# dronefreak/CABiNet

Hardware: NVIDIA B200
Metric: images/sec at 1024x1024 (MNv3-L) (higher is better)
Workload: dtype bf16

## Files before the change

cabinet_b200/_lib.py:

```python

from __future__ import annotations

import ctypes as C
import subprocess
from pathlib import Path

PKG = Path(__file__).resolve().parent
LIB_PATH = PKG / "libcabinet_b200.so"
CSRC = PKG / "csrc"

F32, BF16, F16 = 0, 1, 2
ACT_NONE, ACT_RELU, ACT_HSWISH, ACT_HSIGMOID, ACT_SIGMOID = 0, 1, 2, 3, 4

_p, _i, _ll, _f = C.c_void_p, C.c_int, C.c_longlong, C.c_float

SIGNATURES = {
    "cabinet_last_error": ([], C.c_char_p),
    "cabinet_abi_version": ([], _i),
    "cabinet_device_info": ([C.POINTER(_i)] * 3, _i),
    "cabinet_debug_flags": ([_i], _i),
    "cabinet_debug_read": ([_p, _i], _i),
    "cabinet_conv2d_simt": ([_p, _i, _ll, _ll, _ll, _ll, _ll, _p, _i, _ll, _ll, _ll, _p, _p, _ll, _p, _i, _ll, _ll,
                             _i, _i, _i, _i, _i, _i, _i, _i, _i, _i, _i, _i, _i, _f, _p], _i),
    "cabinet_conv_tc": ([_p, _ll, _i, _i, _i, _i, _p, _i, _i, _i, _i, _i, _p, _p, _ll, _p, _i, _ll, _i, _i, _i, _p], _i),
    "cabinet_conv_tc_dt": ([_p, _ll, _i, _i, _i, _i, _p, _i, _i, _i, _i, _i, _p, _p, _ll, _p, _i, _ll, _i, _i, _i, _i, _p],
                           _i),
    "cabinet_conv_tc_view": ([_p, _ll, _i, _i, _i, _i, _p, _i, _i, _i, _i, _p, _p, _ll, _i, _i, _ll, _ll, _ll, _p], _i),
    "cabinet_conv_tc_view_dt": ([_p, _ll, _i, _i, _i, _i, _p, _i, _i, _i, _i, _p, _p, _ll, _i, _i, _ll, _ll, _ll, _i, _p], _i),
    "cabinet_conv_tc_se": ([_p, _ll, _i, _i, _i, _i, _p, _i, _p, _i, _i, _i, _i, _i, _p, _p, _ll, _p, _i, _ll, _i, _i, _i,
                            _p], _i),
    "cabinet_conv_tc_split_act": ([_p, _ll, _i, _i, _i, _i, _p, _i, _i, _i, _i, _i, _p, _p, _i, _ll, _i, _i, _i, _i, _p], _i),
    "cabinet_conv_tc_imgw": ([_p, _ll, _i, _i, _i, _i, _p, _ll, _i, _i, _i, _i, _i, _p, _p, _ll, _p, _i, _ll, _i, _i, _i,
                              _p], _i),
    "cabinet_conv_tc_imgw_dt": ([_p, _ll, _i, _i, _i, _i, _p, _ll, _i, _i, _i, _i, _i, _p, _p, _ll, _p, _i, _ll, _i, _i, _i,
                                 _i, _p], _i),
    "cabinet_conv_tc_up": ([_p, _ll, _i, _i, _i, _i, _p, _i, _i, _i, _i, _i, _p, _p, _i, _i, _p, _ll, _i, _i, _i, _p], _i),
    "cabinet_gate_scale_weights": ([_p, _i, _f, _p, _p, _p, _p, _i, _i, _i, _p, _p, _i, _i, _i, _i, _i, _p], _i),
    "cabinet_scale_weights": ([_p, _p, _p, _i, _i, _i, _i, _i, _i, _p], _i),
    "cabinet_stem_tc": ([_p, _i, _i, _i, _p, _p, _p, _ll, _p, _ll, _i, _i, _p], _i),
    "cabinet_stem_tc2": ([_p, _i, _i, _i, _p, _p, _ll, _p, _ll, _i, _i, _p], _i),
    "cabinet_dwconv": ([_p, _ll, _p, _p, _p, _ll, _i, _i, _i, _i, _i, _i, _i, _i, _i, _i, _p, _p], _i),
    "cabinet_dwconv_tma": ([_p, _ll, _p, _p, _p, _ll, _i, _i, _i, _i, _i, _i, _i, _i, _i, _p, _p], _i),
    "cabinet_dwconv_tma_dt": ([_p, _ll, _p, _p, _p, _ll, _i, _i, _i, _i, _i, _i, _i, _i, _i, _p, _i, _p], _i),
    "cabinet_mbconv_noexpand_fused": ([_p, _ll, _p, _p, _p, _p, _p, _ll, _i, _i, _i, _i, _i, _p], _i),
    "cabinet_mbconv_fused": ([_p, _ll, _i, _i, _i, _i, _p, _p, _i, _i, _i, _i, _i, _p, _p, _i, _i, _p, _ll, _i, _i, _p,
                              _p], _i),
    "cabinet_mbconv_t": ([_p, _ll, _i, _i, _i, _i, _p, _p, _i, _i, _i, _i, _i, _p, _p, _i, _i, _p, _ll, _i, _i, _p, _p,
                          _p], _i),
    "cabinet_expand_sums": ([_p, _ll, _i, _i, _i, _i, _p, _p, _i, _i, _i, _i, _p, _p], _i),
    "cabinet_gate_mlp": ([_p, _f, _p, _p, _p, _p, _p, _i, _i, _i, _i, _p], _i),
    "cabinet_gate_fc": ([_p, _f, _p, _p, _p, _i, _i, _i, _i, _i, _p], _i),
    "cabinet_scale_act": ([_p, _ll, _i, _p, _i, _ll, _i, _i, _i, _p], _i),
    "cabinet_psp_pool": ([_p, _ll, _i, _p, _i, _i, _i, _i, _p, _ll, _p], _i),
    "cabinet_psp_concat": ([_p, _ll, _p, _p, _ll, _i, _i, _i, _i, _i, _p], _i),
    "cabinet_softmax_rows": ([_p, _p, _i, _ll, _i, _p], _i),
    "cabinet_attention_tc": ([_p, _ll, _p, _ll, _p, _ll, _p, _p, _ll, _i, _i, _i, _f, _p], _i),
    "cabinet_cab_combine": ([_p, _p, _p, _p, _ll, _p, _i, _ll, _i, _p], _i),
    "cabinet_channel_sum": ([_p, _ll, _i, _i, _ll, _i, _p, _p, _ll, _p], _i),
    "cabinet_bilinear_nhwc": ([_p, _ll, _i, _p, _ll, _i, _i, _i, _i, _i, _i, _i, _p], _i),
    "cabinet_upsample_logits_nchw": ([_p, _i, _i, _i, _i, _p, _i, _i, _i, _p], _i),
    "cabinet_upsample_argmax": ([_p, _i, _i, _i, _i, _p, _i, _i, _p, _i, _i, _p, _p], _i),
    "cabinet_normalize_u8": ([_p, _p, _i, _i, _i, _f, _f, _f, _f, _f, _f, _p], _i),
    "cabinet_confusion_hist": ([_p, _i, _p, _i, _ll, _i, _i, _p, _p], _i),
    "cabinet_upsample_softmax_accum": ([_p, _p, _i, _i, _i, _i, _i, _i, _p, _ll, _ll, _ll, _i, _i, _i, _i, _p, _p, _f,
                                        _p], _i),
    "cabinet_prob_resize_accum": ([_p, _i, _i, _i, _i, _i, _i, _i, _i, _p, _i, _i, _p], _i),
    "cabinet_argmax_hist_nchw": ([_p, _i, _i, _ll, _p, _p, _i, _i, _p, _p], _i),
    "cabinet_ohem_workspace_bytes": ([], _ll),
    "cabinet_train_scratch_floats": ([_ll, _i, _i], _ll),
    "cabinet_pack_conv_weight": ([_p, _i, _i, _i, _i, _p, _i, _i, _i, _i, _p], _i),
    "cabinet_pack_conv_weight_parity": ([_p, _i, _i, _i, _i, _i, _i, _i, _i, _i, _p, _i, _i, _p], _i),
    "cabinet_pack_conv_weight_parity_dt": ([_p, _i, _i, _i, _i, _i, _i, _i, _i, _i, _p, _i, _i, _i, _p], _i),
    "cabinet_pack_dw_weight": ([_p, _i, _i, _i, _p, _p], _i),
    "cabinet_im2col_nchw": ([_p, _i, _i, _i, _i, _i, _i, _i, _p, _ll, _p], _i),
    "cabinet_im2col_nchw_dt": ([_p, _i, _i, _i, _i, _i, _i, _i, _p, _ll, _i, _p], _i),
    "cabinet_embed_filter": ([_p, _i, _i, _i, _i, _p, _ll, _i, _p], _i),
    "cabinet_bn_train_stats": ([_p, _ll, _i, _ll, _i, _p, _p, _f, _f, _p, _p, _p, _p, _p], _i),
    "cabinet_affine_act": ([_p, _ll, _i, _p, _p, _p, _f, _p, _ll, _p, _ll, _i, _ll, _ll, _i, _i, _p], _i),
    "cabinet_bn_train_backward": ([_p, _ll, _p, _ll, _i, _p, _i, _p, _p, _p, _ll, _ll, _i, _i, _p, _p], _i),
    "cabinet_bn_frozen_stats": ([_p, _p, _p, _p, _f, _i, _p, _p], _i),
    "cabinet_bn_frozen_backward": ([_p, _ll, _p, _ll, _i, _p, _i, _p, _p, _p, _ll, _ll, _i, _i, _p, _p], _i),
    "cabinet_stem_dgrad": ([_p, _ll, _p, _ll, _i, _p, _p, _p, _i, _i, _i, _i, _i, _p], _i),
    "cabinet_gate_scale_backward": ([_p, _ll, _p, _ll, _i, _p, _f, _i, _p, _i, _ll, _i, _p, _p], _i),
    "cabinet_gate_apply_backward": ([_p, _ll, _p, _ll, _i, _p, _f, _p, _f, _i, _p, _ll, _i, _ll, _i, _i, _p], _i),
    "cabinet_gate_mlp_backward": ([_p, _f, _p, _p, _p, _p, _p, _i, _i, _i, _i, _p, _p, _p, _p, _p, _p, _p], _i),
    "cabinet_col_sum": ([_p, _ll, _i, _ll, _i, _p, _i, _p, _p], _i),
    "cabinet_conv_dgrad": ([_p, _ll, _i, _p, _i, _ll, _ll, _p, _ll, _i, _i, _i, _i, _i, _i, _i, _i, _i, _i, _i, _i, _p], _i),
    "cabinet_conv_wgrad_scratch_floats": ([_i, _i, _i, _i, _i, _i, _i], _ll),
    "cabinet_conv_wgrad": ([_p, _ll, _i, _p, _i, _ll, _ll, _ll, _ll, _p, _i, _i, _i, _i, _i, _i, _i, _i, _i, _i, _i, _p,
                            _p], _i),
    "cabinet_conv_wgrad_tc_scratch_floats": ([_i, _i, _i, _i, _i, _i, _i, _i, _i], _ll),
    "cabinet_conv_wgrad_tc": ([_p, _ll, _p, _ll, _p, _i, _i, _i, _i, _i, _i, _i, _i, _i, _p, _p], _i),
    "cabinet_conv_wgrad_tc_dt": ([_p, _ll, _p, _ll, _p, _i, _i, _i, _i, _i, _i, _i, _i, _i, _p, _i, _p], _i),
# ... 57 lines not shown
```

cabinet_b200/engine.py:

```python

from __future__ import annotations

import math
from dataclasses import dataclass
from typing import Optional

import torch

from . import _lib
from ._lib import ACT_HSIGMOID, ACT_HSWISH, ACT_NONE, ACT_RELU, ACT_SIGMOID, BF16, F16, F32, check
from .constants import BN_EPS


_DTYPE_CODES = {torch.float32: F32, torch.bfloat16: BF16, torch.float16: F16}


def dtype_code(dtype: torch.dtype) -> int:
    code = _DTYPE_CODES.get(dtype)
    if code is None:
        raise TypeError(f"cabinet_b200 kernels take float32, bfloat16 or float16 tensors, got {dtype}")
    return code


@dataclass
# ... 121 lines not shown
    return o


def _out_size(n, k, s, p):
    return (n + 2 * p - k) // s + 1


class Engine:
    PACKED_ATTRS = ("stem", "blocks", "last", "stem_tc", "sb1", "sb2", "sb3", "sb4", "conva", "to_q", "to_k", "to_v",
                    "psp_k", "psp_v", "proj_out", "local", "gamma", "convb", "b1", "b4", "key_ch", "qkv", "ffm_blk",
                    "ffm_gate", "head_conv", "head_out", "ffm_sb", "low_fold", "stem_tc2")

    def __init__(self, model, precision: str = "bf16", packed: Optional[dict] = None):
        if precision not in ("bf16", "fp32"):
            raise ValueError(f"precision must be 'bf16' or 'fp32', got {precision!r}")
        p0 = next(model.parameters())
        if not p0.is_cuda:
            raise RuntimeError("cabinet_b200 engine needs the model on a CUDA device (no CPU path)")
        self.lib = _lib.load()
        self.dev = p0.device
        self.precision = precision
        self.tdt = torch.bfloat16 if precision == "bf16" else torch.float32
        self.dt = BF16 if precision == "bf16" else F32
        self.n_classes = model.n_classes
        self.stamp = None
        self.launches = 0
        self.use_tc = precision == "bf16"
        self.debug = False
        self.stages = {}
        self.trace, self.trace_filter = None, None
        self.fuse_mbconv = True
        self.se_from_sums = True
        self.use_stem2 = True
        self.t_small_s2 = False
        self.t_k5s2 = True
        self.use_mbconv_t = True
        self.fold_se_relu = True
        self.fold_ffm = True
        self.fold_low_up = False
        self.reverse_layers = frozenset()
        self.fuse_se = False
        self.fuse_se_blocks = frozenset({"mobile.f12", "mobile.f13"})
        self.use_cuda_graph = False
        self.sub_batch = 0
        self._graphs = {}
        self._pool = None
        self._graph_seen = {}
        self.dual_stream = False
        self._side = None
        self._scratch = []
        self.branch_overlap = True
        self._branch_streams, self._branch_events = [], {}
        self.sb_overlap = False
        if packed is not None:
            missing = [a for a in self.PACKED_ATTRS if a not in packed]
            if missing:
                raise ValueError(f"packed weights lack {missing}")
            for a in self.PACKED_ATTRS:
                setattr(self, a, _from_plain(packed[a]))
            self.gamma = model.ab.a2block.gamma.detach().float().contiguous()
        else:
            with torch.no_grad():
                self._pack(model)
                for a in self.PACKED_ATTRS:
                    setattr(self, a, _map_tensors(getattr(self, a), lambda t: t.to(self.dev)))

    def packed_state(self) -> dict:
        return {a: _to_plain(getattr(self, a)) for a in self.PACKED_ATTRS}

    def _pack(self, m):
        wd = self.tdt
        f32 = torch.float32
        mob = m.mobile
        self.stem = ConvLayer(mob.features[0][0], mob.features[0][1], ACT_HSWISH, f32, "mobile.stem")
        self.blocks = []
        for bi, blk in enumerate(list(mob.features)[1:], 1):
            s, c = blk.spec, blk.conv
            act = ACT_HSWISH if s["hs"] else ACT_RELU
            e = dict(spec=s, act=act)
            if s["expand"]:
                e["pw1"] = ConvLayer(c[0], c[1], act, wd, f"mobile.f{bi}.expand")
                e["dw"] = DwLayer(c[3], c[4], ACT_NONE if s["se"] else act, f"mobile.f{bi}.dw")
                se, pw2, bn2 = c[5], c[7], c[8]
                if self.precision == "bf16":
                    dwl, kk, nc = e["dw"], e["dw"].k ** 2, -(-e["dw"].c // 64)
                    aux = torch.zeros((nc * 64, kk + 2), dtype=f32, device=dwl.w.device)
                    aux[: dwl.c, :kk] = dwl.w.t()
                    aux[: dwl.c, kk + 1] = dwl.b
                    e["aux"] = aux.view(nc, 64, kk + 2).permute(0, 2, 1).contiguous()
                    p1 = e["pw1"]
                    if p1.cin % 8 == 0 and p1.cin % 64 <= 56 and p1.cin <= 248:
                        wb = torch.zeros((-(-p1.cout // 16) * 16, (p1.cin // 64 + 1) * 64), dtype=f32, device=dwl.w.device)
                        wb[: p1.cout, : p1.cin] = p1.tc[: p1.cout, 0, : p1.cin].float()
                        hi = p1.b.to(torch.bfloat16).float()
                        wb[: p1.cout, p1.cin], wb[: p1.cout, p1.cin + 1] = hi, p1.b - hi
                        e["w1b"] = wb.to(torch.bfloat16).contiguous()
                        ch = 64 if dwl.c <= 64 else 128
                        nct = 1 if dwl.c <= 64 else -(-dwl.c // 128)
                        flat = torch.zeros((nct * ch, wb.shape[1]), dtype=f32, device=dwl.w.device)
                        flat[: dwl.c] = wb[: dwl.c]
                        e["w1t"] = (flat.view(nct, ch, -1).repeat(1, 128 // ch, 1).reshape(nct * 128, -1)
                                    .to(torch.bfloat16).contiguous())
                        fa = torch.zeros((nct * ch, kk + 1), dtype=f32, device=dwl.w.device)
                        fa[: dwl.c, :kk] = dwl.w.t()
                        fa[: dwl.c, kk] = dwl.b
                        e["auxt"] = fa.view(nct, ch, kk + 1).repeat(1, 128 // ch, 1).permute(0, 2, 1).contiguous()
# ... 78 lines not shown
    def _run(self, kernel: str, layer: str, nbytes: int, flops: int, fn, *args):
        nbytes, fused_bytes = nbytes if isinstance(nbytes, tuple) else (nbytes, nbytes)
        tr = self.trace
        if tr is not None and (self.trace_filter is None or kernel in self.trace_filter):
            e0, e1 = torch.cuda.Event(enable_timing=True), torch.cuda.Event(enable_timing=True)
            e0.record()
            rc = fn(*args)
            e1.record()
            tr.append((kernel, layer, nbytes, flops, e0, e1, fused_bytes))
        else:
            rc = fn(*args)
        check(rc, f"{kernel}[{layer}]")
        self.launches += 1

    def new(self, N, H, W, C, dtype=None) -> Map:
        t = torch.empty((N, H, W, C), dtype=dtype or self.tdt, device=self.dev)
        return Map(t, N, H, W, C, C)

    def conv(self, x: Map, L: ConvLayer, out: Optional[Map] = None, res: Optional[Map] = None, out_dtype=None,
             nchw_input: Optional[torch.Tensor] = None, a_scale: Optional[torch.Tensor] = None, a_act: int = 0) -> Map:
        if nchw_input is not None:
            N, _, H, W = nchw_input.shape
            xptr, xdt, xes = nchw_input.data_ptr(), F32, 4
            sxn, sxh, sxw, sxc = 3 * H * W, W, 1, H * W
            cin = 3
        else:
            N, H, W, cin = x.N, x.H, x.W, x.C
            xptr, xdt, xes = x.ptr, x.dt, x.t.element_size()
            sxn, sxh, sxw, sxc = H * W * x.ld, W * x.ld, x.ld, 1
        assert cin == L.cin, (L.name, cin, L.cin)
        OH, OW = _out_size(H, L.kh, L.stride, L.pad), _out_size(W, L.kw, L.stride, L.pad)
        if out is None:
            out = self.new(N, OH, OW, L.cout, out_dtype)
        assert (out.N, out.H, out.W, out.C) == (N, OH, OW, L.cout), L.name
        M = N * OH * OW
        nbytes = (N * H * W * cin * xes + M * L.cout * out.t.element_size() + L.w.numel() * L.w.element_size()
                  + (M * L.cout * res.t.element_size() if res is not None else 0))
        flops = 2 * M * L.cout * L.cin * L.kh * L.kw
        if (self.use_tc and L.tc is not None and nchw_input is None and x.dt == BF16 and x.ld % 8 == 0
                and x.off % 8 == 0 and (L.stride == 1 or (H >= 2 and W >= 2))
                and (out.dt == F32 or (out.ld % 8 == 0 and out.off % 8 == 0))):
            self._conv_tc(x, L, out, res, OH, OW, nbytes, flops, a_scale, a_act)
            return out
        assert a_scale is None, "the SE prologue exists on the tcgen05 path only"
        wdt = BF16 if L.w.dtype == torch.bfloat16 else F32
        self._run("conv2d_simt", L.name, nbytes, flops, self.lib.cabinet_conv2d_simt,
                  xptr, xdt, sxn, sxh, sxw, sxc, 0, L.w.data_ptr(), wdt, L.w.shape[1], 1, 0, L.b.data_ptr(),
                  res.ptr if res is not None else None, res.ld if res is not None else 0,
                  out.ptr, out.dt, out.ld, 0, 1, N, H, W, cin, L.cout, L.kh, L.kw, L.stride, L.pad, OH, OW, L.act,
                  1.0, self.stream)
        return out

    REVERSE_TILES = 0x100

    def _conv_tc(self, x: Map, L: ConvLayer, out: Map, res: Optional[Map], OH, OW, nbytes, flops, a_scale=None, a_act=0):
        self._run("conv_tc", L.name, nbytes, flops, self.lib.cabinet_conv_tc_se, x.ptr, x.ld, x.N, x.H, x.W, x.C,
                  a_scale.data_ptr() if a_scale is not None else None, a_act,
                  L.tc.data_ptr(), L.cout, L.kh, L.kw, L.stride, L.pad, L.b.data_ptr(),
                  res.ptr if res is not None else None, res.ld if res is not None else 0, out.ptr, out.dt, out.ld,
                  OH, OW, L.act | (self.REVERSE_TILES if L.name in self.reverse_layers else 0), self.stream)

    def dwconv(self, x: Map, L: DwLayer, gap: Optional[torch.Tensor] = None):
        p = (L.k - 1) // 2
        OH, OW = _out_size(x.H, L.k, L.stride, p), _out_size(x.W, L.k, L.stride, p)
        out = self.new(x.N, OH, OW, x.C)
        es = x.t.element_size()
        nbytes = x.N * x.C * (x.H * x.W + OH * OW) * es + L.w.numel() * 4
        flops = 2 * x.N * OH * OW * x.C * L.k * L.k
        if self.use_tc and x.dt == BF16 and x.ld % 8 == 0 and x.off % 8 == 0:
            self._run("dwconv_tma", L.name, nbytes, flops, self.lib.cabinet_dwconv_tma, x.ptr, x.ld, L.w.data_ptr(),
                      L.b.data_ptr(), out.ptr, out.ld, x.N, x.H, x.W, x.C, L.k, L.stride, OH, OW,
                      L.act | (self.REVERSE_TILES if L.name in self.reverse_layers else 0),
                      gap.data_ptr() if gap is not None else None, self.stream)
            return out, True
        self._run("dwconv", L.name, nbytes, flops, self.lib.cabinet_dwconv, x.ptr, x.ld, L.w.data_ptr(),
                  L.b.data_ptr(), out.ptr, out.ld, x.dt, x.N, x.H, x.W, x.C, L.k, L.stride, OH, OW, L.act, None,
                  self.stream)
        if gap is not None:
            self.channel_sum(out, gap, L.name)
        return out, False

    def channel_sum(self, x: Map, out: torch.Tensor, name: str, scratch: Optional[torch.Tensor] = None):
        if scratch is None:
            scratch = torch.zeros(128 + x.N * 64 * x.C, dtype=torch.float32, device=self.dev)
            self.launches += 1
        self._run("channel_sum", name, 0, 0, self.lib.cabinet_channel_sum, x.ptr, x.ld, x.dt, x.N, x.H * x.W, x.C,
                  out.data_ptr(), scratch.data_ptr(), scratch.numel() * 4, self.stream)

    class _Branch:

        def __init__(self, eng, i):
            self.eng, self.i = eng, i

        def __enter__(self):
            eng = self.eng
            if not eng.branch_overlap or eng.trace is not None or torch.device(eng.dev).type != "cuda":
                self.ctx = None
                return lambda t: None
            self.main = torch.cuda.current_stream(eng.dev)
            while len(eng._branch_streams) <= self.i:
                eng._branch_streams.append(torch.cuda.Stream(eng.dev))
            side = eng._branch_streams[self.i]
            ev = torch.cuda.Event()
            ev.record(self.main)
            side.wait_event(ev)
            self.ctx = torch.cuda.stream(side)
            self.ctx.__enter__()
            return lambda t: t.record_stream(self.main)

        def __exit__(self, *a):
            if self.ctx is not None:
                eng = self.eng
                ev = torch.cuda.Event()
# ... 116 lines not shown
        cat = self.new(x.N, x.H, x.W, 5 * x.C)
        self._run("psp_concat", L.name, 0, 0, self.lib.cabinet_psp_concat, x.ptr, x.ld, pooled.data_ptr(), cat.ptr,
                  cat.ld, x.dt, x.N, x.H, x.W, x.C, self.stream)
        return self.conv(cat, L)

    def attention(self, q: Map, k: Map, v: Map) -> Map:
        N, Lq, d = q.N, q.H * q.W, q.C
        es = q.t.element_size()
        ctx = self.new(q.N, q.H, q.W, d)
        if self.use_tc and d == 128 and q.dt == BF16 and all(m.ld % 8 == 0 and m.off % 8 == 0 for m in (q, k, v)):
            vt = torch.empty((N, d, -(-Lq // 8) * 8), dtype=torch.bfloat16, device=self.dev)
            self._run("attention_tc", "cab.attention", 4 * N * Lq * d * es, 4 * N * Lq * Lq * d,
                      self.lib.cabinet_attention_tc, q.ptr, q.ld, k.ptr, k.ld, v.ptr, v.ld, vt.data_ptr(), ctx.ptr,
                      ctx.ld, N, Lq, d, float(d) ** -0.5, self.stream)
            self.launches += 1
            return ctx
        s = torch.empty((N, Lq, Lq), dtype=torch.float32, device=self.dev)
        self._run("conv2d_simt", "cab.qk", 2 * N * Lq * d * es, 2 * N * Lq * Lq * d, self.lib.cabinet_conv2d_simt,
                  q.ptr, q.dt, 0, 0, q.ld, 1, Lq * q.ld, k.ptr, k.dt, k.ld, 1, Lq * k.ld, None, None, 0,
                  s.data_ptr(), F32, Lq, Lq * Lq, N, 1, 1, Lq, d, Lq, 1, 1, 1, 0, 1, Lq, ACT_NONE, float(d) ** -0.5,
                  self.stream)
        p = torch.empty((N, Lq, Lq), dtype=self.tdt, device=self.dev)
        self._run("softmax_rows", "cab.softmax", 0, 0, self.lib.cabinet_softmax_rows, s.data_ptr(), p.data_ptr(),
                  self.dt, N * Lq, Lq, self.stream)
        self._run("conv2d_simt", "cab.pv", 2 * N * Lq * d * es, 2 * N * Lq * Lq * d, self.lib.cabinet_conv2d_simt,
                  p.data_ptr(), self.dt, 0, 0, Lq, 1, Lq * Lq, v.ptr, v.dt, 1, v.ld, Lq * v.ld, None, None, 0,
                  ctx.ptr, ctx.dt, ctx.ld, Lq * ctx.ld, N, 1, 1, Lq, Lq, d, 1, 1, 1, 0, 1, Lq, ACT_NONE, 1.0,
                  self.stream)
        return ctx

    def bilinear(self, x: Map, out: Map, name: str):
        nbytes = x.N * x.C * (x.H * x.W * x.t.element_size() + out.H * out.W * out.t.element_size())
        self._run("bilinear_nhwc", name, nbytes, 0, self.lib.cabinet_bilinear_nhwc, x.ptr, x.ld, x.dt, out.ptr, out.ld,
                  out.dt, x.N, x.H, x.W, x.C, out.H, out.W, self.stream)

    def _trunk(self, x: torch.Tensor, need_aux: bool = True):
        if x.dtype != torch.float32 or not x.is_contiguous():
            x = x.float().contiguous()
        if x.device != self.dev:
            raise RuntimeError(f"input on {x.device}, model on {self.dev}")
        N, _, H, W = x.shape
        self.launches = 0
        dev, C = self.dev, self.n_classes
        n_se = sum(1 for b in self.blocks if "se" in b)
        kc = self.key_ch
        n_gap, n_psp, n_ffm = (2 * n_se + 1) * N * 1024, 128 + N * (110 + 256 * kc), 128 + N * 64 * 256
        zeros_all = torch.zeros(n_gap + 2 * n_psp + n_ffm, dtype=torch.float32, device=dev)
        gap_all = zeros_all[:n_gap].view(2 * n_se + 1, N * 1024)
        self._scratch = [zeros_all[n_gap + i * n_psp: n_gap + (i + 1) * n_psp] for i in range(2)]
        ffm_scratch = zeros_all[n_gap + 2 * n_psp:]
        self.launches += 1

        fused_stems = self.use_tc and self.stem_tc is not None and W % 4 == 0
        if fused_stems:
            OH2, OW2 = (H - 1) // 2 + 1, (W - 1) // 2 + 1
            s1, f0 = self.new(N, OH2, OW2, 64), self.new(N, OH2, OW2, 16)
            nbytes = x.numel() * 4 + (s1.t.numel() + f0.t.numel()) * 2 + 80 * 192 * 2
            if self.use_stem2 and self.stem_tc2 is not None:
                self._run("stem_tc", "sb.conv1+mobile.stem", nbytes, 2 * N * OH2 * OW2 * (64 * 147 + 16 * 27),
                          self.lib.cabinet_stem_tc2, x.data_ptr(), N, H, W, self.stem_tc2.data_ptr(), s1.ptr, s1.ld,
                          f0.ptr, f0.ld, OH2, OW2, self.stream)
            else:
                self._run("stem_tc", "sb.conv1+mobile.stem", nbytes, 2 * N * OH2 * OW2 * (64 * 147 + 16 * 27),
                          self.lib.cabinet_stem_tc, x.data_ptr(), N, H, W, self.stem_tc[0].data_ptr(),
                          self.stem_tc[1].data_ptr(), s1.ptr, s1.ld, f0.ptr, f0.ld, OH2, OW2, self.stream)
        else:
            s1 = self.conv(None, self.sb1, nchw_input=x)
        H8, W8 = _out_size(_out_size(s1.H, 3, 2, 1), 3, 2, 1), _out_size(_out_size(s1.W, 3, 2, 1), 3, 2, 1)
        fold_low = (self.fold_low_up and self.use_tc and not self.debug and self.ffm_sb is not None
                    and self.ffm_sb.tc is not None and self.low_fold.tc is not None and self.sb4.cout == self.ffm_sb.cin)
        cat_ffm = self.new(N, H8, W8, self.sb4.cout if fold_low else 128 + 256)
        if self.sb_overlap:
            with self._branch(2) as joined:
                s2 = self.conv(s1, self.sb2)
                s3 = self.conv(s2, self.sb3)
                self.conv(s3, self.sb4, out=cat_ffm.slice(0, 128))
                joined(s1.t)
        else:
            s2 = self.conv(s1, self.sb2)
            s3 = self.conv(s2, self.sb3)
            self.conv(s3, self.sb4, out=cat_ffm.slice(0, 128))
        assert (s3.H, s3.W) == (H8, W8)

        f = f0 if fused_stems else self.conv(None, self.stem, nchw_input=x)
        gi = 0
        for e in self.blocks:
            s = e["spec"]
            if "fused_pw" in e and self.use_tc and f.ld % 8 == 0 and f.off % 8 == 0:
                o = self.new(f.N, f.H, f.W, s["out"])
                dw = e["dw"]
                es = f.t.element_size()
                self._run("mbconv_noexpand_fused", dw.name.replace(".dw", ""), 2 * f.N * f.H * f.W * f.C * es,
                          2 * f.N * f.H * f.W * f.C * (9 + f.C), self.lib.cabinet_mbconv_noexpand_fused, f.ptr, f.ld,
                          dw.w.data_ptr(), dw.b.data_ptr(), e["fused_pw"][0].data_ptr(), e["fused_pw"][1].data_ptr(),
                          o.ptr, o.ld, f.N, f.H, f.W, f.C, dw.act, self.stream)
                f = o
                continue
            fuse = (s["expand"] and self.fuse_mbconv and self.use_tc and f.dt == BF16 and f.ld % 8 == 0
                    and f.off % 8 == 0 and s["exp"] % 8 == 0 and ("se" in e or s["out"] <= 160) and "w1b" in e
                    and not e.get("nofuse")
                    and not (s["k"] == 5 and s["s"] == 2 and not (self.use_mbconv_t and self.t_k5s2 and "se" in e)))
            d = None
            gap_fixed = False
            if fuse and "se" in e and self.se_from_sums and self._se_from_sums_ok(f, e):
                try:
                    f = self.se_block_one_kernel(f, e, gap_all[2 * gi:2 * gi + 2].view(-1)[: 2 * N * s["exp"]])
                    gi += 1
                    continue
                except ValueError as err:
                    if "budget" not in str(err):
                        raise
                    e["no_sums"] = True
            if fuse:
                gap = None
                if "se" in e:
                    gap, gap_fixed = gap_all[2 * gi:2 * gi + 2].view(-1)[: 2 * N * s["exp"]], True
                pw2l = e["pw2"]
                fold_se = ("se" in e and self.fold_se_relu and e["act"] == ACT_RELU and not self.debug
                           and pw2l.tc is not None and pw2l.kh == 1 and (f.H // s["s"]) * (f.W // s["s"]) % 128 == 0
                           and f.H % s["s"] == 0 and f.W % s["s"] == 0)
                try:
                    d = self.mbconv_fused(f, e, gap, ACT_RELU if fold_se else None)
                except ValueError as err:
                    if "budget" not in str(err):
                        raise
                    e["nofuse"], fuse = True, False
            if fuse and "se" not in e:
                f = d
                continue
            h = self.conv(f, e["pw1"]) if s["expand"] and not fuse else f
            if "se" in e:
                if not fuse:
                    gap = gap_all[2 * gi:2 * gi + 2].view(-1)[: 2 * N * s["exp"]]
                    d, gap_fixed = self.dwconv(h, e["dw"], gap)
                gi += 1
# ... 293 lines not shown
```

include/cabinet_b200.h:

```cpp
#ifndef CABINET_B200_H
#define CABINET_B200_H

#include <stdint.h>

#ifdef __cplusplus
extern "C" {
#endif

#define CABINET_ABI_VERSION 2

enum { CABINET_OK = 0, CABINET_ERR_INVALID = 1, CABINET_ERR_CUDA = 2 };
enum { CABINET_F32 = 0, CABINET_BF16 = 1, CABINET_F16 = 2 };
enum {
    CABINET_ACT_NONE = 0,
    CABINET_ACT_RELU = 1,
    CABINET_ACT_HSWISH = 2,
    CABINET_ACT_HSIGMOID = 3,
    CABINET_ACT_SIGMOID = 4
};
#define CABINET_CONV_REVERSE_TILES 0x100

#define CABINET_GAP_FIXED_ONE 16777216.0f

typedef void* cabinet_stream_t;

const char* cabinet_last_error(void);
int cabinet_abi_version(void);
int cabinet_device_info(int* sm_count, int* cc_major, int* cc_minor);
int cabinet_debug_flags(int flags);
int cabinet_debug_read(long long* host_out, int n);

int cabinet_conv2d_simt(const void* x, int x_dtype, long long sxn, long long sxh, long long sxw, long long sxc,
                        long long x_batch_stride,
                        const void* w, int w_dtype, long long w_sco, long long w_sk, long long w_batch_stride,
                        const float* bias,
                        const void* res, long long ldres,
                        void* y, int y_dtype, long long ldy, long long y_batch_stride,
                        int batches, int N, int H, int W, int Cin, int Cout, int KH, int KW, int stride, int pad,
                        int OH, int OW, int act, float alpha, cabinet_stream_t stream);

int cabinet_conv_tc(const void* x, long long ldx, int N, int H, int W, int Cin, const void* w_packed, int Cout,
                    int KH, int KW, int stride, int pad, const float* bias, const void* res, long long ldres,
                    void* y, int y_dtype, long long ldy, int OH, int OW, int act, cabinet_stream_t stream);
int cabinet_conv_tc_dt(const void* x, long long ldx, int N, int H, int W, int Cin, const void* w_packed, int Cout,
                       int KH, int KW, int stride, int pad, const float* bias, const void* res, long long ldres,
                       void* y, int y_dtype, long long ldy, int OH, int OW, int act, int op_dtype, cabinet_stream_t stream);

int cabinet_conv_tc_view(const void* x, long long ldx, int N, int H, int W, int Cin, const void* w_packed, int Cout, int KH,
                         int KW, int pad, const float* bias, void* y, long long ldy, int OH, int OW, long long y_sw,
                         long long y_sh, long long y_sn, cabinet_stream_t stream);
int cabinet_conv_tc_view_dt(const void* x, long long ldx, int N, int H, int W, int Cin, const void* w_packed, int Cout, int KH,
                            int KW, int pad, const float* bias, void* y, long long ldy, int OH, int OW, long long y_sw,
                            long long y_sh, long long y_sn, int op_dtype, cabinet_stream_t stream);

int cabinet_conv_tc_se(const void* x, long long ldx, int N, int H, int W, int Cin, const float* a_scale, int a_act,
                       const void* w_packed, int Cout, int KH, int KW, int stride, int pad, const float* bias,
                       const void* res, long long ldres, void* y, int y_dtype, long long ldy, int OH, int OW, int act,
                       cabinet_stream_t stream);

int cabinet_stem_tc(const float* x, int N, int H, int W, const void* w_packed, const float* bias, void* y_sb,
                    long long ld_sb, void* y_stem, long long ld_stem, int OH, int OW, cabinet_stream_t stream);

int cabinet_stem_tc2(const float* x, int N, int H, int W, const void* w_packed2, void* y_sb, long long ld_sb, void* y_stem,
                     long long ld_stem, int OH, int OW, cabinet_stream_t stream);

int cabinet_dwconv(const void* x, long long ldx, const float* w, const float* bias, void* y, long long ldy,
                   int dtype, int N, int H, int W, int C, int k, int stride, int OH, int OW, int act,
                   float* gap_sum, cabinet_stream_t stream);

int cabinet_dwconv_tma(const void* x, long long ldx, const float* w, const float* bias, void* y, long long ldy, int N,
                       int H, int W, int C, int k, int stride, int OH, int OW, int act, long long* gap_sum,
                       cabinet_stream_t stream);
int cabinet_dwconv_tma_dt(const void* x, long long ldx, const float* w, const float* bias, void* y, long long ldy, int N,
                          int H, int W, int C, int k, int stride, int OH, int OW, int act, long long* gap_sum, int op_dtype,
                          cabinet_stream_t stream);

int cabinet_mbconv_noexpand_fused(const void* x, long long ldx, const float* w_dw, const float* b_dw,
                                  const float* w_pw, const float* b_pw, void* y, long long ldy, int N, int H, int W,
                                  int C, int act, cabinet_stream_t stream);

int cabinet_conv_tc_up(const void* x, long long ldx, int N, int H, int W, int Cin, const void* w_packed, int Cout,
                       int KH, int KW, int stride, int pad, const float* bias, const float* up, int up_h, int up_w,
                       void* y, long long ldy, int OH, int OW, int act, cabinet_stream_t stream);

int cabinet_conv_tc_split_act(const void* x, long long ldx, int N, int H, int W, int Cin, const void* w_packed, int Cout,
                              int KH, int KW, int stride, int pad, const float* bias, void* y, int y_dtype, long long ldy,
                              int OH, int OW, int act, int act_cols, cabinet_stream_t stream);

int cabinet_conv_tc_imgw(const void* x, long long ldx, int N, int H, int W, int Cin, const void* w_packed_per_image,
                         long long w_image_stride, int Cout, int KH, int KW, int stride, int pad, const float* bias,
                         const void* res, long long ldres, void* y, int y_dtype, long long ldy, int OH, int OW, int act,
                         cabinet_stream_t stream);
int cabinet_conv_tc_imgw_dt(const void* x, long long ldx, int N, int H, int W, int Cin, const void* w_packed_per_image,
                            long long w_image_stride, int Cout, int KH, int KW, int stride, int pad, const float* bias,
                            const void* res, long long ldres, void* y, int y_dtype, long long ldy, int OH, int OW, int act,
                            int op_dtype, cabinet_stream_t stream);

int cabinet_scale_weights(const void* w_packed, const float* scale, void* out, int N, int rows, int taps, int cin_pad,
                          int Cin, int plus_one, cabinet_stream_t stream);

int cabinet_gate_scale_weights(const void* gap_sum, int in_fixed, float inv_hw, const float* w1, const float* b1,
                               const float* w2, const float* b2, int gate, int C, int Cmid, const void* w_packed, void* out,
                               int N, int rows, int taps, int cin_pad, int plus_one, cabinet_stream_t stream);

int cabinet_mbconv_fused(const void* x, long long ldx, int N, int H, int W, int Cin, const void* w_expand,
                         const float* aux_packed, int Cexp, int act_expand, int k, int stride, int act_dw,
                         const void* w_project, const float* b_project, int Cout, int residual, void* y, long long ldy,
                         int OH, int OW, long long* gap_sum, cabinet_stream_t stream);

int cabinet_mbconv_t(const void* x, long long ldx, int N, int H, int W, int Cin, const void* w_expand_t, const float* aux_t,
                     int Cexp, int act_expand, int k, int stride, int act_dw, const void* w_project,
                     const float* b_project, int Cout, int residual, void* y, long long ldy, int OH, int OW,
                     long long* gap_sum, const float* se_scale, cabinet_stream_t stream);

int cabinet_expand_sums(const void* x, long long ldx, int N, int H, int W, int Cin, const void* w_expand_t,
                        const float* aux_t, int Cexp, int act_expand, int k, int nsplit, long long* gap_sum,
                        cabinet_stream_t stream);
// ... 167 lines not shown
```

Before: 6305.

## Fuse spatial-branch conv3 and 1x1 conv_out into one tcgen05 kernel; chunk stem by L2

Adds a persistent tcgen05 kernel that computes the stride-2 3x3 conv (via four parity-split TMA maps) and the following 1x1 conv in one pass. The intermediate stays in TMEM and shared memory, so it is never written to or read back from HBM. The spatial-branch stem and its tail are also processed in batch chunks sized to about half of L2, so the large stem output stays cache-resident between kernels. This costs more launches per chunk, a complex warp-specialized pipeline with a fixed channel configuration, and a stem scratch buffer reused across chunks.

```diff
diff --git a/cabinet_b200/_lib.py b/cabinet_b200/_lib.py
--- a/cabinet_b200/_lib.py
+++ b/cabinet_b200/_lib.py
@@ -39,6 +39,7 @@
     "cabinet_scale_weights": ([_p, _p, _p, _i, _i, _i, _i, _i, _i, _p], _i),
     "cabinet_stem_tc": ([_p, _i, _i, _i, _p, _p, _p, _ll, _p, _ll, _i, _i, _p], _i),
     "cabinet_stem_tc2": ([_p, _i, _i, _i, _p, _p, _ll, _p, _ll, _i, _i, _p], _i),
+    "cabinet_sb_tail_tc": ([_p, _ll, _i, _i, _i, _p, _p, _p, _p, _p, _ll, _i, _i, _p], _i),
     "cabinet_dwconv": ([_p, _ll, _p, _p, _p, _ll, _i, _i, _i, _i, _i, _i, _i, _i, _i, _i, _p, _p], _i),
     "cabinet_dwconv_tma": ([_p, _ll, _p, _p, _p, _ll, _i, _i, _i, _i, _i, _i, _i, _i, _i, _p, _p], _i),
     "cabinet_dwconv_tma_dt": ([_p, _ll, _p, _p, _p, _ll, _i, _i, _i, _i, _i, _i, _i, _i, _i, _p, _i, _p], _i),
diff --git a/cabinet_b200/csrc/sb_tail_tc.cu b/cabinet_b200/csrc/sb_tail_tc.cu
--- /dev/null
+++ b/cabinet_b200/csrc/sb_tail_tc.cu
@@ -0,0 +1,300 @@
+#include "tc_common.cuh"
+
+namespace {
+
+constexpr int BLOCK_M = 128, CIN = 64, CMID = 64, COUT = 128, TAPS = 9;
+constexpr int A_STAGE_BYTES = BLOCK_M * CIN * 2;
+constexpr int W3_TAP_BYTES = CMID * CIN * 2;
+constexpr int W3_BYTES = TAPS * W3_TAP_BYTES;
+constexpr int W4_BYTES = COUT * CMID * 2;
+constexpr int A4_BYTES = BLOCK_M * CMID * 2;
+constexpr int C_BYTES = BLOCK_M * 128;
+constexpr int STAGES = 5;
+constexpr int NUM_THREADS = 192;
+constexpr int SMEM_BYTES = W3_BYTES + W4_BYTES + A4_BYTES + 2 * C_BYTES + STAGES * A_STAGE_BYTES + 1024;
+constexpr int TMEM_COLS = 512;
+constexpr int ACC3_COL = 0, ACC4_COL = 2 * CMID;
+
+struct SbTailParams {
+    int OH, OW, TW, TH, tiles_w, tiles_h, num_tiles;
+    const float* b3;
+    const float* b4;
+};
+
+__device__ __forceinline__ void store_row_sw128(uint32_t tile, int row, const float* v) {
+#pragma unroll
+    for (int c = 0; c < 8; ++c) {
+        uint32_t w[4];
+#pragma unroll
+        for (int j = 0; j < 4; ++j)
+            asm("cvt.rn.relu.bf16x2.f32 %0, %1, %2;" : "=r"(w[j]) : "f"(v[8 * c + 2 * j + 1]), "f"(v[8 * c + 2 * j]));
+        tc::sts128(tile + row * 128 + ((c ^ (row & 7)) << 4), make_uint4(w[0], w[1], w[2], w[3]));
+    }
+}
+
+__global__ void __launch_bounds__(NUM_THREADS, 1)
+sb_tail_tc_kernel(const __grid_constant__ CUtensorMap tmA0, const __grid_constant__ CUtensorMap tmA1,
+                  const __grid_constant__ CUtensorMap tmA2, const __grid_constant__ CUtensorMap tmA3,
+                  const __grid_constant__ CUtensorMap tmW3, const __grid_constant__ CUtensorMap tmW4,
+                  const __grid_constant__ CUtensorMap tmY, const SbTailParams p) {
+    extern __shared__ uint8_t smem_raw[];
+    __shared__ __align__(8) uint64_t full_bar[STAGES], empty_bar[STAGES], w_bar;
+    __shared__ __align__(8) uint64_t acc3_full[2], acc3_empty[2], acc4_full[2], acc4_empty[2], a4_full, a4_empty;
+    __shared__ uint32_t tmem_base_smem;
+    __shared__ __align__(16) float s_b3[CMID];
+    __shared__ __align__(16) float s_b4[COUT];
+
+    uint8_t* smem = reinterpret_cast<uint8_t*>((reinterpret_cast<uintptr_t>(smem_raw) + 1023) & ~uintptr_t(1023));
+    uint8_t* sW3 = smem;
+    uint8_t* sW4 = sW3 + W3_BYTES;
+    uint8_t* sA4 = sW4 + W4_BYTES;
+    uint8_t* sC = sA4 + A4_BYTES;
+    uint8_t* sA = sC + 2 * C_BYTES;
+
+    const int warp = threadIdx.x >> 5, lane = threadIdx.x & 31;
+
+    if (threadIdx.x == 0) {
+        tc::prefetch_tmap(&tmA0);
+        tc::prefetch_tmap(&tmW3);
+        tc::prefetch_tmap(&tmY);
+        for (int s = 0; s < STAGES; ++s) {
+            tc::mbar_init(&full_bar[s], 1);
+            tc::mbar_init(&empty_bar[s], 1);
+        }
+        for (int s = 0; s < 2; ++s) {
+            tc::mbar_init(&acc3_full[s], 1);
+            tc::mbar_init(&acc3_empty[s], 4);
+            tc::mbar_init(&acc4_full[s], 1);
+            tc::mbar_init(&acc4_empty[s], 4);
+        }
+        tc::mbar_init(&a4_full, 4);
+        tc::mbar_init(&a4_empty, 1);
+        tc::mbar_init(&w_bar, 1);
+        tc::mbar_fence_init();
+        tc::fence_proxy_async();
+    }
+    if (threadIdx.x >= 64) {
+        const int t = threadIdx.x - 64;
+        if (t < CMID) s_b3[t] = __ldg(p.b3 + t);
+        s_b4[t] = __ldg(p.b4 + t);
+    }
+    if (warp == 1) tc::tmem_alloc(&tmem_base_smem, TMEM_COLS);
+    tc::tc_fence_before();
+    __syncthreads();
+    tc::tc_fence_after();
+    const uint32_t tmem = tmem_base_smem;
+    const int tiles_per_img = p.tiles_w * p.tiles_h;
+
+    if (warp == 0) {
+        if (lane == 0) {
+            tc::mbar_expect_tx(&w_bar, W3_BYTES + W4_BYTES);
+            for (int t = 0; t < TAPS; ++t) tc::tma_load_2d(sW3 + t * W3_TAP_BYTES, &tmW3, &w_bar, t * CIN, 0);
+            tc::tma_load_2d(sW4, &tmW4, &w_bar, 0, 0);
+            int s = 0;
+            uint32_t ph = 0;
+            for (int tile = blockIdx.x; tile < p.num_tiles; tile += gridDim.x) {
+                const int img = tile / tiles_per_img, r = tile - img * tiles_per_img;
+                const int oh0 = (r / p.tiles_w) * p.TH, ow0 = (r % p.tiles_w) * p.TW;
+#pragma unroll 1
+                for (int t = 0; t < TAPS; ++t) {
+                    tc::mbar_wait(&empty_bar[s], ph ^ 1);
+                    tc::mbar_expect_tx(&full_bar[s], A_STAGE_BYTES);
+                    const int ty = t / 3 - 1, tx = t % 3 - 1;
+                    const int py = ty & 1, px = tx & 1;
+                    const int id = py * 2 + px;
+                    const CUtensorMap* map = id == 0 ? &tmA0 : id == 1 ? &tmA1 : id == 2 ? &tmA2 : &tmA3;
+                    tc::tma_load_4d(sA + s * A_STAGE_BYTES, map, &full_bar[s], 0, ow0 + ((tx - px) >> 1),
+                                    oh0 + ((ty - py) >> 1), img);
+                    if (++s == STAGES) { s = 0; ph ^= 1; }
+                }
+            }
+        }
+        __syncwarp();
+    } else if (warp == 1) {
+        const uint32_t leader = tc::elect_one();
+        const uint32_t idesc3 = tc::make_idesc_bf16(BLOCK_M, CMID), idesc4 = tc::make_idesc_bf16(BLOCK_M, COUT);
+        const uint64_t a_desc0 = tc::make_desc_sw128(tc::smem_u32(sA));
+        const uint64_t w3_desc0 = tc::make_desc_sw128(tc::smem_u32(sW3));
+        const uint64_t a4_desc = tc::make_desc_sw128(tc::smem_u32(sA4));
+        const uint64_t w4_desc = tc::make_desc_sw128(tc::smem_u32(sW4));
+        tc::mbar_wait(&w_bar, 0);
+        int s = 0, it = 0;
+        uint32_t ph = 0;
+        auto issue_out = [&](int j) {
+            const int acc = j & 1;
+            tc::mbar_wait(&a4_full, j & 1);
+            tc::mbar_wait(&acc4_empty[acc], ((j >> 1) & 1) ^ 1);
+            tc::tc_fence_after();
+            const uint32_t d = tmem + ACC4_COL + acc * COUT;
+#pragma unroll
+            for (int k = 0; k < CMID / 16; ++k) tc::umma_bf16_if(leader, d, a4_desc + 2 * k, w4_desc + 2 * k, idesc4, k ? 1u : 0u);
+            tc::umma_commit_if(leader, &a4_empty);
+            tc::umma_commit_if(leader, &acc4_full[acc]);
+        };
+        for (int tile = blockIdx.x; tile < p.num_tiles; tile += gridDim.x, ++it) {
+            const int acc = it & 1;
+            tc::mbar_wait(&acc3_empty[acc], ((it >> 1) & 1) ^ 1);
+            tc::tc_fence_after();
+            const uint32_t d = tmem + ACC3_COL + acc * CMID;
+#pragma unroll 1
+            for (int t = 0; t < TAPS; ++t) {
+                tc::mbar_wait(&full_bar[s], ph);
+                tc::tc_fence_after();
+                const uint64_t a_desc = a_desc0 + static_cast<uint64_t>(s * (A_STAGE_BYTES >> 4));
+                const uint64_t b_desc = w3_desc0 + static_cast<uint64_t>(t * (W3_TAP_BYTES >> 4));
+#pragma unroll
+                for (int k = 0; k < CIN / 16; ++k)
+                    tc::umma_bf16_if(leader, d, a_desc + 2 * k, b_desc + 2 * k, idesc3, (t | k) ? 1u : 0u);
+                tc::umma_commit_if(leader, &empty_bar[s]);
+                if (++s == STAGES) { s = 0; ph ^= 1; }
+            }
+            tc::umma_commit_if(leader, &acc3_full[acc]);
+            if (it > 0) issue_out(it - 1);
+        }
+        if (it > 0) issue_out(it - 1);
+        __syncwarp();
+    } else {
+        const int q = warp & 3;
+        const int row = q * 32 + lane;
+        const bool leader = warp == 2 && lane == 0;
+        const uint32_t lane_off = static_cast<uint32_t>(q * 32) << 16;
+        int it = 0;
+        for (int tile = blockIdx.x; tile < p.num_tiles; tile += gridDim.x, ++it) {
+            const int img = tile / tiles_per_img, r = tile - img * tiles_per_img;
+            const int oh0 = (r / p.tiles_w) * p.TH, ow0 = (r % p.tiles_w) * p.TW;
+            const int acc = it & 1;
+            tc::mbar_wait(&acc3_full[acc], (it >> 1) & 1);
+            tc::tc_fence_after();
+            {
+                uint32_t v[64];
+                tc::tmem_ld32(tmem + ACC3_COL + acc * CMID + lane_off, v);
+                tc::tmem_ld32(tmem + ACC3_COL + acc * CMID + 32 + lane_off, v + 32);
+                tc::tmem_ld_wait();
+                tc::tc_fence_before();
+                __syncwarp();
+                if (lane == 0) tc::mbar_arrive(&acc3_empty[acc]);
+                float f[64];
+#pragma unroll
+                for (int j = 0; j < 64; ++j) f[j] = __uint_as_float(v[j]) + s_b3[j];
+                tc::mbar_wait(&a4_empty, (it & 1) ^ 1);
+                store_row_sw128(tc::smem_u32(sA4), row, f);
+                tc::fence_proxy_async();
+                __syncwarp();
+                if (lane == 0) tc::mbar_arrive(&a4_full);
+            }
+            tc::mbar_wait(&acc4_full[acc], (it >> 1) & 1);
+            tc::tc_fence_after();
+            if (leader) tc::bulk_wait_read<0>();
+            tc::named_bar_sync(1, 128);
+#pragma unroll 1
+            for (int g = 0; g < 2; ++g) {
+                uint32_t v[64];
+                tc::tmem_ld32(tmem + ACC4_COL + acc * COUT + g * 64 + lane_off, v);
+                tc::tmem_ld32(tmem + ACC4_COL + acc * COUT + g * 64 + 32 + lane_off, v + 32);
+                tc::tmem_ld_wait();
+                float f[64];
+#pragma unroll
+                for (int j = 0; j < 64; ++j) f[j] = __uint_as_float(v[j]) + s_b4[g * 64 + j];
+                store_row_sw128(tc::smem_u32(sC + g * C_BYTES), row, f);
+            }
+            tc::tc_fence_before();
+            __syncwarp();
+            if (lane == 0) tc::mbar_arrive(&acc4_empty[acc]);
+            tc::fence_proxy_async();
+            tc::named_bar_sync(1, 128);
+            if (leader) {
+                tc::tma_store_4d(&tmY, sC, 0, ow0, oh0, img);
+                tc::tma_store_4d(&tmY, sC + C_BYTES, 64, ow0, oh0, img);
+                tc::bulk_commit();
+            }
+        }
+        if (leader) tc::bulk_wait_read<0>();
+    }
+    tc::tc_fence_before();
+    __syncthreads();
+    if (warp == 1) {
+        tc::tc_fence_after();
+        tc::tmem_dealloc(tmem, TMEM_COLS);
+    }
+}
+
+bool g_attr_set = false;
+
+}
+
+extern "C" int cabinet_sb_tail_tc(const void* x, long long ldx, int N, int H, int W, const void* w3_packed,
+                                  const float* b3, const void* w4_packed, const float* b4, void* y, long long ldy, int OH,
+                                  int OW, cabinet_stream_t stream) {
+    CAB_REQUIRE(x && w3_packed && b3 && w4_packed && b4 && y, "sb_tail_tc: null pointer");
+    CAB_REQUIRE(N >= 0 && H >= 2 && W >= 2, "sb_tail_tc: the stride-2 conv needs H, W >= 2");
+    CAB_REQUIRE(OH == (H - 1) / 2 + 1 && OW == (W - 1) / 2 + 1, "sb_tail_tc: inconsistent output size");
+    CAB_REQUIRE(ldx >= CIN && ldx % 8 == 0 && (reinterpret_cast<uintptr_t>(x) & 15) == 0,
+                "sb_tail_tc: input needs 16-byte aligned pixels (ldx %% 8 == 0)");
+    CAB_REQUIRE(ldy >= COUT && ldy % 8 == 0 && (reinterpret_cast<uintptr_t>(y) & 15) == 0,
+                "sb_tail_tc: output needs 16-byte aligned pixels (ldy %% 8 == 0)");
+    CAB_REQUIRE((reinterpret_cast<uintptr_t>(w3_packed) & 15) == 0 && (reinterpret_cast<uintptr_t>(w4_packed) & 15) == 0,
+                "sb_tail_tc: weight alignment");
+    if (N == 0) return CABINET_OK;
+
+    SbTailParams p;
+    p.OH = OH; p.OW = OW; p.b3 = b3; p.b4 = b4;
+    long long best = -1;
+    for (int tw = 128; tw >= 4; tw >>= 1) {
+        const int th = BLOCK_M / tw;
+        const long long cover = cab_ceil_div(OW, tw) * tw * cab_ceil_div(OH, th) * th;
+        if (best < 0 || cover < best) { best = cover; p.TW = tw; p.TH = th; }
+    }
+    p.tiles_w = static_cast<int>(cab_ceil_div(OW, p.TW));
+    p.tiles_h = static_cast<int>(cab_ceil_div(OH, p.TH));
+    const long long nt = static_cast<long long>(N) * p.tiles_w * p.tiles_h;
+    CAB_REQUIRE(nt < (1LL << 31), "sb_tail_tc: too many tiles");
+    p.num_tiles = static_cast<int>(nt);
+
+    const uint64_t es = 2;
+    CUtensorMap tmA[4], tmW3, tmW4, tmY;
+    {
+        const uint32_t box[4] = {CIN, (uint32_t)p.TW, (uint32_t)p.TH, 1};
+        const uint16_t* xb = reinterpret_cast<const uint16_t*>(x);
+        for (int py = 0; py < 2; ++py)
+            for (int px = 0; px < 2; ++px) {
+                const uint64_t dims[4] = {(uint64_t)CIN, (uint64_t)((W - px + 1) / 2), (uint64_t)((H - py + 1) / 2), (uint64_t)N};
+                const uint64_t strides[3] = {(uint64_t)ldx * es * 2, (uint64_t)ldx * es * W * 2, (uint64_t)ldx * es * W * H};
+                int rc = cab_make_tmap_bf16(&tmA[py * 2 + px], xb + (static_cast<long long>(py) * W + px) * ldx, 4, dims,
+                                            strides, box);
+                if (rc) return rc;
+            }
+    }
+    {
+        const uint64_t dims[2] = {(uint64_t)TAPS * CIN, (uint64_t)CMID};
+        const uint64_t strides[1] = {(uint64_t)TAPS * CIN * es};
+        const uint32_t box[2] = {CIN, CMID};
+        int rc = cab_make_tmap_bf16(&tmW3, w3_packed, 2, dims, strides, box, CU_TENSOR_MAP_L2_PROMOTION_L2_256B);
+        if (rc) return rc;
+    }
+    {
+        const uint64_t dims[2] = {(uint64_t)CMID, (uint64_t)COUT};
+        const uint64_t strides[1] = {(uint64_t)CMID * es};
+        const uint32_t box[2] = {CMID, COUT};
+        int rc = cab_make_tmap_bf16(&tmW4, w4_packed, 2, dims, strides, box, CU_TENSOR_MAP_L2_PROMOTION_L2_256B);
+        if (rc) return rc;
+    }
+    {
+        const uint64_t dims[4] = {(uint64_t)COUT, (uint64_t)OW, (uint64_t)OH, (uint64_t)N};
+        const uint64_t strides[3] = {(uint64_t)ldy * es, (uint64_t)ldy * es * OW, (uint64_t)ldy * es * OW * OH};
+        const uint32_t box[4] = {64, (uint32_t)p.TW, (uint32_t)p.TH, 1};
+        int rc = cab_make_tmap_bf16(&tmY, y, 4, dims, strides, box);
+        if (rc) return rc;
+    }
+    if (!g_attr_set) {
+        CAB_CUDA(cudaFuncSetAttribute(sb_tail_tc_kernel, cudaFuncAttributeMaxDynamicSharedMemorySize, SMEM_BYTES));
+        g_attr_set = true;
+    }
+    int dev = 0, sms = 148;
+    CAB_CUDA(cudaGetDevice(&dev));
+    CAB_CUDA(cudaDeviceGetAttribute(&sms, cudaDevAttrMultiProcessorCount, dev));
+    const int grid = static_cast<int>(std::min<long long>(nt, sms));
+    sb_tail_tc_kernel<<<grid, NUM_THREADS, SMEM_BYTES, static_cast<cudaStream_t>(stream)>>>(tmA[0], tmA[1], tmA[2], tmA[3],
+                                                                                            tmW3, tmW4, tmY, p);
+    CAB_LAUNCH_CHECK();
+    return CABINET_OK;
+}
diff --git a/cabinet_b200/engine.py b/cabinet_b200/engine.py
--- a/cabinet_b200/engine.py
+++ b/cabinet_b200/engine.py
@@ -197,6 +197,9 @@
         self.branch_overlap = True
         self._branch_streams, self._branch_events = [], {}
         self.sb_overlap = False
+        self.fuse_sb_tail = True
+        self.sb_group = 0
+        self._l2_bytes = None
         if packed is not None:
             missing = [a for a in self.PACKED_ATTRS if a not in packed]
             if missing:
@@ -381,6 +384,7 @@
         return out
 
     REVERSE_TILES = 0x100
+    SB_GROUP_L2_SHARE = 0.5
 
     def _conv_tc(self, x: Map, L: ConvLayer, out: Map, res: Optional[Map], OH, OW, nbytes, flops, a_scale=None, a_act=0):
         self._run("conv_tc", L.name, nbytes, flops, self.lib.cabinet_conv_tc_se, x.ptr, x.ld, x.N, x.H, x.W, x.C,
@@ -388,6 +392,42 @@
                   L.tc.data_ptr(), L.cout, L.kh, L.kw, L.stride, L.pad, L.b.data_ptr(),
                   res.ptr if res is not None else None, res.ld if res is not None else 0, out.ptr, out.dt, out.ld,
                   OH, OW, L.act | (self.REVERSE_TILES if L.name in self.reverse_layers else 0), self.stream)
+
+    def _sb_group(self, N, OH2, OW2) -> int:
+        if self.sb_group > 0:
+            return min(self.sb_group, N)
+        if self._l2_bytes is None:
+            self._l2_bytes = (torch.cuda.get_device_properties(self.dev).L2_cache_size if self.dev.type == "cuda"
+                              else 0)
+        g = int(self._l2_bytes * self.SB_GROUP_L2_SHARE) // (OH2 * OW2 * 64 * 2)
+        return g if 1 <= g < N else N
+
+    def _sb_tail_fusable(self, s2: Map, out: Map) -> bool:
+        L3, L4 = self.sb3, self.sb4
+        return (self.fuse_sb_tail and self.use_tc and not self.debug and L3.tc is not None and L4.tc is not None
+                and (L3.cin, L3.cout, L3.kh, L3.kw, L3.stride, L3.pad) == (64, 64, 3, 3, 2, 1)
+                and (L4.cin, L4.cout, L4.kh, L4.kw, L4.stride, L4.pad) == (64, 128, 1, 1, 1, 0)
+                and s2.dt == BF16 and s2.C == 64 and s2.ld % 8 == 0 and s2.off % 8 == 0 and s2.H >= 2 and s2.W >= 2
+                and out.dt == BF16 and out.ld % 8 == 0 and out.off % 8 == 0
+                and not any(n.startswith("sb.") for n in self.reverse_layers))
+
+    def _sb_rest(self, s1: Map, out: Map):
+        s2 = self.conv(s1, self.sb2)
+        if not self._sb_tail_fusable(s2, out):
+            s3 = self.conv(s2, self.sb3)
+            self.conv(s3, self.sb4, out=out)
+            return
+        L3, L4 = self.sb3, self.sb4
+        N, H, W = s2.N, s2.H, s2.W
+        OH, OW = _out_size(H, 3, 2, 1), _out_size(W, 3, 2, 1)
+        assert (out.N, out.H, out.W, out.C) == (N, OH, OW, 128)
+        M, wbytes = N * OH * OW, (L3.w.numel() + L4.w.numel()) * 2
+        layer_bytes = N * H * W * 64 * 2 + 2 * M * 64 * 2 + M * 128 * 2 + wbytes
+        fused_bytes = N * H * W * 64 * 2 + M * 128 * 2 + wbytes
+        flops = 2 * M * 64 * 64 * 9 + 2 * M * 128 * 64
+        self._run("sb_tail_tc", "sb.conv3+sb.conv_out", (layer_bytes, fused_bytes), flops, self.lib.cabinet_sb_tail_tc,
+                  s2.ptr, s2.ld, N, H, W, L3.tc.data_ptr(), L3.b.data_ptr(), L4.tc.data_ptr(), L4.b.data_ptr(),
+                  out.ptr, out.ld, OH, OW, self.stream)
 
     def dwconv(self, x: Map, L: DwLayer, gap: Optional[torch.Tensor] = None):
         p = (L.k - 1) // 2
@@ -610,35 +650,44 @@
         self.launches += 1
 
         fused_stems = self.use_tc and self.stem_tc is not None and W % 4 == 0
-        if fused_stems:
-            OH2, OW2 = (H - 1) // 2 + 1, (W - 1) // 2 + 1
-            s1, f0 = self.new(N, OH2, OW2, 64), self.new(N, OH2, OW2, 16)
-            nbytes = x.numel() * 4 + (s1.t.numel() + f0.t.numel()) * 2 + 80 * 192 * 2
-            if self.use_stem2 and self.stem_tc2 is not None:
-                self._run("stem_tc", "sb.conv1+mobile.stem", nbytes, 2 * N * OH2 * OW2 * (64 * 147 + 16 * 27),
-                          self.lib.cabinet_stem_tc2, x.data_ptr(), N, H, W, self.stem_tc2.data_ptr(), s1.ptr, s1.ld,
-                          f0.ptr, f0.ld, OH2, OW2, self.stream)
-            else:
-                self._run("stem_tc", "sb.conv1+mobile.stem", nbytes, 2 * N * OH2 * OW2 * (64 * 147 + 16 * 27),
-                          self.lib.cabinet_stem_tc, x.data_ptr(), N, H, W, self.stem_tc[0].data_ptr(),
-                          self.stem_tc[1].data_ptr(), s1.ptr, s1.ld, f0.ptr, f0.ld, OH2, OW2, self.stream)
-        else:
-            s1 = self.conv(None, self.sb1, nchw_input=x)
-        H8, W8 = _out_size(_out_size(s1.H, 3, 2, 1), 3, 2, 1), _out_size(_out_size(s1.W, 3, 2, 1), 3, 2, 1)
+        OH2, OW2 = (H - 1) // 2 + 1, (W - 1) // 2 + 1
+        H8, W8 = _out_size(_out_size(OH2, 3, 2, 1), 3, 2, 1), _out_size(_out_size(OW2, 3, 2, 1), 3, 2, 1)
         fold_low = (self.fold_low_up and self.use_tc and not self.debug and self.ffm_sb is not None
                     and self.ffm_sb.tc is not None and self.low_fold.tc is not None and self.sb4.cout == self.ffm_sb.cin)
         cat_ffm = self.new(N, H8, W8, self.sb4.cout if fold_low else 128 + 256)
-        if self.sb_overlap:
-            with self._branch(2) as joined:
-                s2 = self.conv(s1, self.sb2)
-                s3 = self.conv(s2, self.sb3)
-                self.conv(s3, self.sb4, out=cat_ffm.slice(0, 128))
-                joined(s1.t)
+        if fused_stems:
+            f0 = self.new(N, OH2, OW2, 16)
+            g = N if self.sb_overlap else self._sb_group(N, OH2, OW2)
+            s1 = self.new(g, OH2, OW2, 64)
+            for n0 in range(0, N, g):
+                nc = min(g, N - n0)
+                s1c = Map(s1.t[:nc], nc, OH2, OW2, 64, 64)
+                f0c = Map(f0.t[n0:n0 + nc], nc, OH2, OW2, 16, 16)
+                xc = x[n0:n0 + nc]
+                nbytes = xc.numel() * 4 + nc * OH2 * OW2 * (64 + 16) * 2 + 80 * 192 * 2
+                flops = 2 * nc * OH2 * OW2 * (64 * 147 + 16 * 27)
+                if self.use_stem2 and self.stem_tc2 is not None:
+                    self._run("stem_tc", "sb.conv1+mobile.stem", nbytes, flops, self.lib.cabinet_stem_tc2, xc.data_ptr(),
+                              nc, H, W, self.stem_tc2.data_ptr(), s1c.ptr, s1c.ld, f0c.ptr, f0c.ld, OH2, OW2, self.stream)
+                else:
+                    self._run("stem_tc", "sb.conv1+mobile.stem", nbytes, flops, self.lib.cabinet_stem_tc, xc.data_ptr(),
+                              nc, H, W, self.stem_tc[0].data_ptr(), self.stem_tc[1].data_ptr(), s1c.ptr, s1c.ld, f0c.ptr,
+                              f0c.ld, OH2, OW2, self.stream)
+                out = Map(cat_ffm.t[n0:n0 + nc], nc, H8, W8, 128, cat_ffm.ld)
+                if self.sb_overlap:
+                    with self._branch(2) as joined:
+                        self._sb_rest(s1c, out)
+                        joined(s1.t)
+                else:
+                    self._sb_rest(s1c, out)
         else:
-            s2 = self.conv(s1, self.sb2)
-            s3 = self.conv(s2, self.sb3)
-            self.conv(s3, self.sb4, out=cat_ffm.slice(0, 128))
-        assert (s3.H, s3.W) == (H8, W8)
+            s1 = self.conv(None, self.sb1, nchw_input=x)
+            if self.sb_overlap:
+                with self._branch(2) as joined:
+                    self._sb_rest(s1, cat_ffm.slice(0, 128))
+                    joined(s1.t)
+            else:
+                self._sb_rest(s1, cat_ffm.slice(0, 128))
 
         f = f0 if fused_stems else self.conv(None, self.stem, nchw_input=x)
         gi = 0
diff --git a/include/cabinet_b200.h b/include/cabinet_b200.h
--- a/include/cabinet_b200.h
+++ b/include/cabinet_b200.h
@@ -63,6 +63,10 @@
 
 int cabinet_stem_tc2(const float* x, int N, int H, int W, const void* w_packed2, void* y_sb, long long ld_sb, void* y_stem,
                      long long ld_stem, int OH, int OW, cabinet_stream_t stream);
+
+int cabinet_sb_tail_tc(const void* x, long long ldx, int N, int H, int W, const void* w3_packed, const float* b3,
+                       const void* w4_packed, const float* b4, void* y, long long ldy, int OH, int OW,
+                       cabinet_stream_t stream);
 
 int cabinet_dwconv(const void* x, long long ldx, const float* w, const float* bias, void* y, long long ldy,
                    int dtype, int N, int H, int W, int C, int k, int stride, int OH, int OW, int act,
```

After: 5820, median of 6. 0.923x the previous value.
